# tinganchen/AlignQ

Hardware: AMD Instinct MI355X
Metric: images/sec (train step, CDF+ADMM) ResNet-20 8-bit (higher is better)
Workload: dtype f32; 1 GPU; resnet20 CIFAR-shape 3x32x32, 8W/8A CDF+ADMM full train step (cdf_alignment_admm/resnet-20-cifar-10), batch 128/GPU, HIP-graph replay, batch-norm folded into the site kernels, channels-last tensors, all Conv2d_Q convolutions on alignq_conv*_nhwc (exact-product bf16 MFMA); global_batch=128, parallelism=dp1

## Files before the change

alignq_amd/csrc/conv_kernels.hip:

```cpp
#include <hip/hip_runtime.h>
#include <stdint.h>
#include <stdlib.h>

#include "../../include/alignq.h"
#include "site_internal.h"
#include "store_forms.h"
#include "wgrad_reduce_body.h"

namespace {

using namespace alignq_wgr;

typedef __bf16 bf16x8 __attribute__((ext_vector_type(8)));
typedef __bf16 bf16x4 __attribute__((ext_vector_type(4)));
typedef float f32x4 __attribute__((ext_vector_type(4)));
typedef short s16x4 __attribute__((ext_vector_type(4)));

#ifdef ALIGNQ_STAMPS
__device__ unsigned long long g_conv_stamps[64];
__device__ unsigned long long g_conv_blk[2][4096];
#define STAMP(on, i)                                                          \
  do {                                                                        \
    if ((on) && threadIdx.x == 0) g_conv_stamps[i] = wall_clock64();          \
  } while (0)
#define BSTAMP(which)                                                                          \
  do {                                                                                         \
    if (threadIdx.x == 0 && blockIdx.x < 4096) g_conv_blk[which][blockIdx.x] = wall_clock64(); \
  } while (0)
#else
#define STAMP(on, i) do { } while (0)
#define BSTAMP(which) do { } while (0)
#endif

__device__ __forceinline__ s16x4 tr_read(const __bf16* p) {
  return __builtin_amdgcn_ds_read_tr16_b64_v4i16((__attribute__((address_space(3))) s16x4*)(p));
}
__device__ __forceinline__ bf16x8 join8(s16x4 a, s16x4 b) {
  typedef short s16x8 __attribute__((ext_vector_type(8)));
  s16x8 v = {a[0], a[1], a[2], a[3], b[0], b[1], b[2], b[3]};
  return __builtin_bit_cast(bf16x8, v);
}


template <int xb>
__device__ __forceinline__ f32x4 fetch_act4(const float* __restrict__ x, int64_t off) {
  if constexpr (xb == 0) return *reinterpret_cast<const f32x4*>(x + off);
  if constexpr (xb == 2) {
    const s16x4 b = *reinterpret_cast<const s16x4*>(reinterpret_cast<const short*>(x) + off);
    return (f32x4){(float)b[0], (float)b[1], (float)b[2], (float)b[3]};
  }
  const char4 b = *reinterpret_cast<const char4*>(reinterpret_cast<const signed char*>(x) + off);
  return (f32x4){(float)b.x, (float)b.y, (float)b.z, (float)b.w};
}

struct BnLazy {
  const float* z;
  const float* ab;
  const float* save;
  const float* ktot;
  const float* part = nullptr;
  int n_tiles = 0, tile_f = 0;
  double inv_n = 1.0;
  float* dgamma = nullptr;
  float* dbeta = nullptr;
};

template <int C>
__device__ __forceinline__ void bn_totals_lds(const BnLazy& t, float* __restrict__ kt, bool publish) {
  static_assert(256 % C == 0, "thread -> (channel, group)");
  __shared__ double red[256][2];
  constexpr int G = 256 / C;
  const int tid = threadIdx.x;
  const int cp = C < t.tile_f ? C : t.tile_f;
  const int cyc = C / cp, cnt = t.n_tiles / cyc;
  const int c = tid % C, grp = tid / C;
  const int e = c % cp, t_first = c / cp;
  double s0 = 0, s1 = 0;
  constexpr int U = 16;
  for (int i0 = grp; i0 < cnt; i0 += G * U) {
    float2 v[U];
#pragma unroll
    for (int u = 0; u < U; u++) {
      const int i = i0 + u * G;
      const int ic = i < cnt ? i : cnt - 1;
      v[u] = *reinterpret_cast<const float2*>(t.part + ((int64_t)(ic * cyc + t_first) * cp + e) * 2);
    }
#pragma unroll
    for (int u = 0; u < U; u++) {
      if (i0 + u * G < cnt) { s0 += v[u].x; s1 += v[u].y; }
    }
  }
  red[tid][0] = s0;
  red[tid][1] = s1;
  __syncthreads();
  if (tid < C) {
    double t0 = 0, t1 = 0;
#pragma unroll
    for (int g = 0; g < G; g++) { t0 += red[g * C + tid][0]; t1 += red[g * C + tid][1]; }
    kt[tid] = (float)(t0 * t.inv_n);
    kt[C + tid] = (float)(t1 * t.inv_n);
    if (publish) {
      if (t.dbeta) t.dbeta[tid] = (float)t0;
      if (t.dgamma) t.dgamma[tid] = (float)t1;
    }
  }
  __syncthreads();
}

__device__ __forceinline__ float4 bn_lazy4(const float4& g, const float4& z, const float4& a, const float4& m, const float4& is,
                                           const float4& k0, const float4& k1) {
  float4 o;
  o.x = a.x * (g.x - k0.x - (z.x - m.x) * is.x * k1.x);
  o.y = a.y * (g.y - k0.y - (z.y - m.y) * is.y * k1.y);
  o.z = a.z * (g.z - k0.z - (z.z - m.z) * is.z * k1.z);
  o.w = a.w * (g.w - k0.w - (z.w - m.w) * is.w * k1.w);
  return o;
}

template <int C> constexpr int conv_cp() { return C == 16 ? 16 : (C == 32 ? 48 : C + 8); }
template <int C, int WD, int PT>
struct ConvLds {
  static constexpr int kBf16 = 3 * ((PT / WD) + 2) * (WD + 2) * conv_cp<C>();
};

template <int C, int WD, int PT, bool DGRAD, int XB = 0, bool IMG = false>
__device__ __forceinline__ void conv3x3_body(const float* __restrict__ x, const float* __restrict__ w,
                                             float* __restrict__ y, int H, int total_rows, float nlev, __bf16* lds,
                                             int block, const float* __restrict__ add,
                                             float* __restrict__ bn_part = nullptr, int n_wg = 0,
                                             BnLazy lazy = BnLazy{nullptr, nullptr, nullptr, nullptr}, float xlev = 1.0f) {
  static_assert(XB == 0 || !DGRAD, "the data gradient reads fp32 dy");
  constexpr int xb = XB;
  constexpr int TR = PT / WD;
  constexpr int NS = (9 * C + 31) / 32;
  constexpr int NCG = C / 16;
  constexpr int NPP = 4 / NCG;
  constexpr int NG = PT / 16;
  constexpr int LW = WD + 2;
  constexpr int CP = conv_cp<C>();
  constexpr int LROWS = TR + 2;
  constexpr int ARR = LROWS * LW * CP;
  static_assert(3 * ARR == ConvLds<C, WD, PT>::kBf16, "LDS size");
  __bf16* Xhi = lds;
  __bf16* Xmi = lds + ARR;
  __bf16* Xlo = lds + 2 * ARR;

  const int tid = threadIdx.x, lane = tid & 63, wv = tid >> 6;
  const int row0 = block * TR;
  const int img_lo = (row0 / H) * H, img_hi = img_lo + H;
  [[maybe_unused]] constexpr int SB = DGRAD ? 8 : 0;
  STAMP(block == 0, SB + 0);
  const int cog = wv % NCG, pp = wv / NCG;
  const int m = lane & 15, q = lane >> 4;
  bf16x8 ab[NS];
  {
    constexpr int C4 = C / 4;
    constexpr int N4 = LROWS * LW * C4;
    constexpr int NIT = (N4 + 255) / 256;
    float4 v[NIT];
#pragma unroll
    for (int it = 0; it < NIT; it++) {
      const int i = tid + 256 * it;
      const int c4 = i % C4, col = (i / C4) % LW, lr = i / (C4 * LW);
      const int grow = row0 + lr - 1;
      const bool ok = i < N4 && col >= 1 && col <= WD && grow >= img_lo && grow < img_hi && grow < total_rows;
      const int64_t off = ok ? ((int64_t)grow * WD + (col - 1)) * C + 4 * c4 : 0;
      const f32x4 ld = fetch_act4<XB>(x, off);
      v[it] = ok ? make_float4(ld[0], ld[1], ld[2], ld[3]) : make_float4(0.f, 0.f, 0.f, 0.f);
    }
    STAMP(block == 0, SB + 1);
    if (DGRAD && lazy.z) {
      float4 zz[NIT];
#pragma unroll
      for (int it = 0; it < NIT; it++) {
        const int i = tid + 256 * it;
        const int c4 = i % C4, col = (i / C4) % LW, lr = i / (C4 * LW);
        const int grow = row0 + lr - 1;
        const bool ok = i < N4 && col >= 1 && col <= WD && grow >= img_lo && grow < img_hi && grow < total_rows;
        zz[it] = *reinterpret_cast<const float4*>(lazy.z + (ok ? ((int64_t)grow * WD + (col - 1)) * C + 4 * c4 : 0));
      }
      const int c4t = tid % C4;
      const float4 a4 = *reinterpret_cast<const float4*>(lazy.ab + 4 * c4t);
      const float4 m4 = *reinterpret_cast<const float4*>(lazy.save + 4 * c4t);
      const float4 i4 = *reinterpret_cast<const float4*>(lazy.save + C + 4 * c4t);
      float4 k0, k1;
      if (lazy.part) {
        __shared__ __attribute__((aligned(16))) float kt[2 * C];
        bn_totals_lds<C>(lazy, kt, block == 0);
        k0 = *reinterpret_cast<const float4*>(kt + 4 * c4t);
        k1 = *reinterpret_cast<const float4*>(kt + C + 4 * c4t);
      } else {
        k0 = *reinterpret_cast<const float4*>(lazy.ktot + 4 * c4t);
        k1 = *reinterpret_cast<const float4*>(lazy.ktot + C + 4 * c4t);
      }
#pragma unroll
      for (int it = 0; it < NIT; it++) {
        const int i = tid + 256 * it;
        const int col = (i / C4) % LW, lr = i / (C4 * LW);
        const int grow = row0 + lr - 1;
        const bool ok = i < N4 && col >= 1 && col <= WD && grow >= img_lo && grow < img_hi && grow < total_rows;
        if (ok) v[it] = bn_lazy4(v[it], zz[it], a4, m4, i4, k0, k1);
      }
    }
#pragma unroll
    for (int it = 0; it < NIT; it++) {
      const int i = tid + 256 * it;
      if (i < N4) {
        const int c4 = i % C4, col = (i / C4) % LW, lr = i / (C4 * LW);
        bf16x4 h4, m4, l4;
        const float vv[4] = {v[it].x, v[it].y, v[it].z, v[it].w};
#pragma unroll
        for (int e = 0; e < 4; e++) {
          const __bf16 hi = (__bf16)vv[e];
          const float r1 = vv[e] - (float)hi;
          const __bf16 mi = (__bf16)r1;
          const float r2 = r1 - (float)mi;
          h4[e] = hi; m4[e] = mi; l4[e] = (__bf16)r2;
        }
        const int o = (lr * LW + col) * CP + 4 * c4;
        *reinterpret_cast<bf16x4*>(Xhi + o) = h4;
        *reinterpret_cast<bf16x4*>(Xmi + o) = m4;
        *reinterpret_cast<bf16x4*>(Xlo + o) = l4;
      }
    }
    STAMP(block == 0, SB + 2);
    if constexpr (IMG) {
      const bf16x8* __restrict__ wi = reinterpret_cast<const bf16x8*>(w) + (cog * NS) * 64 + lane;
#pragma unroll
      for (int s = 0; s < NS; s++) ab[s] = wi[s * 64];
    } else {
#pragma unroll
      for (int s = 0; s < NS; s++) {
        const int k0 = 32 * s + 8 * q;
        const bool live = k0 / C < 9;
        const int tap = live ? k0 / C : 8, c0 = k0 % C;
        float wr[8];
        if (!DGRAD) {
          const float* p = w + ((int64_t)(cog * 16 + m) * 9 + tap) * C + c0;
          const float4 a4 = *reinterpret_cast<const float4*>(p), b4 = *reinterpret_cast<const float4*>(p + 4);
          wr[0] = a4.x; wr[1] = a4.y; wr[2] = a4.z; wr[3] = a4.w; wr[4] = b4.x; wr[5] = b4.y; wr[6] = b4.z; wr[7] = b4.w;
        } else {
#pragma unroll
          for (int j = 0; j < 8; j++) wr[j] = w[((int64_t)(c0 + j) * 9 + (8 - tap)) * C + cog * 16 + m];
        }
#pragma unroll
        for (int j = 0; j < 8; j++) ab[s][j] = (__bf16)rintf((live ? wr[j] : 0.f) * nlev);
      }
    }
    STAMP(block == 0, SB + 3);
  }
  __syncthreads();
  constexpr int GW = NG / NPP;
  static_assert(NG % NPP == 0, "every wave takes the same number of pixel groups");
  int bo[GW];
  f32x4 acc[GW];
#pragma unroll
  for (int gi = 0; gi < GW; gi++) {
    const int p = (pp + gi * NPP) * 16 + (lane & 15);
    bo[gi] = ((p / WD) * LW + (p % WD)) * CP;
    acc[gi] = (f32x4){0.f, 0.f, 0.f, 0.f};
  }
  constexpr int GB = (DGRAD && GW > 2) ? 2 : GW;
  static_assert(GW % GB == 0, "whole batches of groups");
#pragma unroll
  for (int g0 = 0; g0 < GW; g0 += GB) {
    bf16x8 bh[2][GB], bm[2][GB], bl[2][GB];
#pragma unroll
    for (int s = 0; s <= NS; s++) {
      if (s < NS) {
        const int k0 = 32 * s + 8 * q;
        const bool live = k0 / C < 9;
        const int tap = live ? k0 / C : 8, c0 = k0 % C;
        const int to = ((tap / 3) * LW + (tap % 3)) * CP + c0;
#pragma unroll
        for (int gi = 0; gi < GB; gi++) {
          const int o = bo[g0 + gi] + to;
          bh[s & 1][gi] = *reinterpret_cast<const bf16x8*>(Xhi + o);
          bm[s & 1][gi] = *reinterpret_cast<const bf16x8*>(Xmi + o);
          if (DGRAD || xb == 0) bl[s & 1][gi] = *reinterpret_cast<const bf16x8*>(Xlo + o);
          if ((9 * C) % 32 != 0 && !live) {
#pragma unroll
            for (int j = 0; j < 8; j++) { bh[s & 1][gi][j] = (__bf16)0.f; bm[s & 1][gi][j] = (__bf16)0.f; bl[s & 1][gi][j] = (__bf16)0.f; }
          }
        }
      }
      __builtin_amdgcn_sched_barrier(0);
      if (s > 0) {
        const int u = s - 1;
#pragma unroll
        for (int gi = 0; gi < GB; gi++) {
          f32x4 a = acc[g0 + gi];
          if (DGRAD || xb == 0) a = __builtin_amdgcn_mfma_f32_16x16x32_bf16(ab[u], bl[u & 1][gi], a, 0, 0, 0);
          a = __builtin_amdgcn_mfma_f32_16x16x32_bf16(ab[u], bm[u & 1][gi], a, 0, 0, 0);
          acc[g0 + gi] = __builtin_amdgcn_mfma_f32_16x16x32_bf16(ab[u], bh[u & 1][gi], a, 0, 0, 0);
        }
      }
    }
  }
  float bs[4] = {0.f, 0.f, 0.f, 0.f}, bq[4] = {0.f, 0.f, 0.f, 0.f};
#pragma unroll
  for (int gi = 0; gi < GW; gi++) {
    const int p = (pp + gi * NPP) * 16 + (lane & 15);
    const int r = p / WD, c = p % WD;
    const int grow = row0 + r;
    if (grow < total_rows) {
      const int64_t o = ((int64_t)grow * WD + c) * C + cog * 16 + 4 * q;
      const float den = (!DGRAD && xb != 0) ? nlev * xlev : nlev;
      float4 v = make_float4(acc[gi][0] / den, acc[gi][1] / den, acc[gi][2] / den, acc[gi][3] / den);
      if (add) {
        const float4 r = *reinterpret_cast<const float4*>(add + o);
        v.x += r.x; v.y += r.y; v.z += r.z; v.w += r.w;
      }
      alignq_store::st16<alignq_store::kConvOut>(y + o, v);
      bs[0] += v.x; bs[1] += v.y; bs[2] += v.z; bs[3] += v.w;
      bq[0] += v.x * v.x; bq[1] += v.y * v.y; bq[2] += v.z * v.z; bq[3] += v.w * v.w;
    }
  }
  STAMP(block == 0, SB + 4);
  if (!DGRAD && bn_part) {
    float* red = reinterpret_cast<float*>(lds);
#define ROW_SHR_ADD(V, CTRL) V += __builtin_bit_cast(float, __builtin_amdgcn_update_dpp(0, __builtin_bit_cast(int, V), CTRL, 0xf, 0xf, false))
#pragma unroll
    for (int e = 0; e < 4; e++) {
      ROW_SHR_ADD(bs[e], 0x111); ROW_SHR_ADD(bs[e], 0x112); ROW_SHR_ADD(bs[e], 0x114); ROW_SHR_ADD(bs[e], 0x118);
      ROW_SHR_ADD(bq[e], 0x111); ROW_SHR_ADD(bq[e], 0x112); ROW_SHR_ADD(bq[e], 0x114); ROW_SHR_ADD(bq[e], 0x118);
    }
#undef ROW_SHR_ADD
    __syncthreads();
    if ((lane & 15) == 15) {
#pragma unroll
      for (int e = 0; e < 4; e++) {
        red[(wv * 16 + 4 * q + e) * 2] = bs[e];
        red[(wv * 16 + 4 * q + e) * 2 + 1] = bq[e];
      }
    }
    __syncthreads();
    if (tid < C) {
      const int cg = tid / 16, cl = tid % 16;
      float s0 = 0.f, s1 = 0.f;
#pragma unroll
      for (int ppi = 0; ppi < NPP; ppi++) {
        const int w2 = ppi * NCG + cg;
        s0 += red[(w2 * 16 + cl) * 2];
        s1 += red[(w2 * 16 + cl) * 2 + 1];
      }
      bn_part[((int64_t)tid * n_wg + block) * 2] = s0;
      bn_part[((int64_t)tid * n_wg + block) * 2 + 1] = s1;
    }
  }
  STAMP(block == 0, SB + 5);
}

template <int C, int WD, int PT, bool DGRAD, int XB = 0, bool IMG = false>
__global__ __launch_bounds__(256) void conv3x3_nhwc_kernel(const float* __restrict__ x, const float* __restrict__ w,
                                                           float* __restrict__ y, int H, int total_rows, float nlev,
                                                           const float* __restrict__ add, float* __restrict__ bn_part,
                                                           float xlev) {
  __shared__ __attribute__((aligned(16))) __bf16 lds[ConvLds<C, WD, PT>::kBf16];
  conv3x3_body<C, WD, PT, DGRAD, XB, IMG>(x, w, y, H, total_rows, nlev, lds, blockIdx.x, add, bn_part, gridDim.x,
                                          BnLazy{nullptr, nullptr, nullptr, nullptr}, xlev);
}

template <int CIN, int COUT, int WDI, int KS, int S, int PT>
struct ConvGen {
  static constexpr int WDO = WDI / S, TR = PT / WDO;
  static constexpr int LROWS = KS == 3 ? TR * S + (S == 1 ? 2 : 1) : TR;
  static constexpr int LW = KS == 3 ? WDI + 2 : WDO;
  static constexpr int CP = CIN + 8;
  static constexpr int ARR = LROWS * LW * CP;
};

template <int CIN, int COUT, int WDI, int KS, int S, int PT, bool IMG = false>
__device__ __forceinline__ void convgen_fwd_body(const float* __restrict__ x, const float* __restrict__ w,
                                                 float* __restrict__ y, int H, int total_rows, float nlev,
                                                 float* __restrict__ bn_part, __bf16* lds, int block, int n_wg) {
  using G = ConvGen<CIN, COUT, WDI, KS, S, PT>;
  constexpr int WDO = G::WDO, TR = G::TR, LROWS = G::LROWS, LW = G::LW, CP = G::CP, ARR = G::ARR;
  constexpr int NS = (KS * KS * CIN + 31) / 32;
  constexpr int NCG = COUT / 16, NPP = 4 / NCG, NG = PT / 16;
  static_assert(NCG == 1 || NCG == 2 || NCG == 4, "output channels");
  __bf16* Xhi = lds;
  __bf16* Xmi = lds + ARR;
  __bf16* Xlo = lds + 2 * ARR;
  const int tid = threadIdx.x, lane = tid & 63, wv = tid >> 6;
  const int row0 = block * TR;
  const int Hin = H * S;
  const int img_lo = (row0 / H) * Hin, img_hi = img_lo + Hin;
  const int cog = wv % NCG, pp = wv / NCG;
  const int m = lane & 15, q = lane >> 4;
  bf16x8 ab[NS];
  {
    constexpr int C4 = CIN / 4;
    constexpr int N4 = LROWS * LW * C4;
    constexpr int NIT = (N4 + 255) / 256;
    float4 v[NIT];
#pragma unroll
    for (int it = 0; it < NIT; it++) {
      const int i = tid + 256 * it;
      const int c4 = i % C4, col = (i / C4) % LW, lr = i / (C4 * LW);
      int grow, gcol;
      if (KS == 3) { grow = row0 * S - 1 + lr; gcol = col - 1; }
      else { grow = (row0 + lr) * S; gcol = col * S; }
      const bool ok = i < N4 && gcol >= 0 && gcol < WDI && grow >= img_lo && grow < img_hi;
      v[it] = *reinterpret_cast<const float4*>(x + (ok ? ((int64_t)grow * WDI + gcol) * CIN + 4 * c4 : 0));
      if (!ok) v[it] = make_float4(0.f, 0.f, 0.f, 0.f);
    }
#pragma unroll
    for (int it = 0; it < NIT; it++) {
      const int i = tid + 256 * it;
      if (i < N4) {
        const int c4 = i % C4, col = (i / C4) % LW, lr = i / (C4 * LW);
        bf16x4 h4, m4, l4;
        const float vv[4] = {v[it].x, v[it].y, v[it].z, v[it].w};
#pragma unroll
        for (int e = 0; e < 4; e++) {
          const __bf16 hi = (__bf16)vv[e];
          const float r1 = vv[e] - (float)hi;
          const __bf16 mi = (__bf16)r1;
          h4[e] = hi; m4[e] = mi; l4[e] = (__bf16)(r1 - (float)mi);
        }
        const int o = (lr * LW + col) * CP + 4 * c4;
        *reinterpret_cast<bf16x4*>(Xhi + o) = h4;
        *reinterpret_cast<bf16x4*>(Xmi + o) = m4;
        *reinterpret_cast<bf16x4*>(Xlo + o) = l4;
      }
    }
    if constexpr (IMG) {
      const bf16x8* __restrict__ wi = reinterpret_cast<const bf16x8*>(w) + (cog * NS) * 64 + lane;
#pragma unroll
      for (int s = 0; s < NS; s++) ab[s] = wi[s * 64];
    } else {
#pragma unroll
      for (int s = 0; s < NS; s++) {
        const int k0 = 32 * s + 8 * q;
        const bool live = k0 / CIN < KS * KS;
        const int tap = live ? k0 / CIN : KS * KS - 1, c0 = k0 % CIN;
        const float* p = w + ((int64_t)(cog * 16 + m) * (KS * KS) + tap) * CIN + c0;
        const float4 a4 = *reinterpret_cast<const float4*>(p), b4 = *reinterpret_cast<const float4*>(p + 4);
        const float wr[8] = {a4.x, a4.y, a4.z, a4.w, b4.x, b4.y, b4.z, b4.w};
#pragma unroll
        for (int j = 0; j < 8; j++) ab[s][j] = (__bf16)rintf((live ? wr[j] : 0.f) * nlev);
      }
    }
  }
  __syncthreads();
  constexpr int GW = NG / NPP;
  static_assert(NG % NPP == 0, "every wave takes the same number of pixel groups");
  int bo[GW];
  f32x4 acc[GW];
#pragma unroll
  for (int gi = 0; gi < GW; gi++) {
    const int p = (pp + gi * NPP) * 16 + (lane & 15);
    const int r = p / WDO, c = p % WDO;
    bo[gi] = (KS == 3 ? (r * S * LW + c * S) : (r * LW + c)) * CP;
    acc[gi] = (f32x4){0.f, 0.f, 0.f, 0.f};
  }
  bf16x8 bh[2][GW], bm[2][GW], bl[2][GW];
#pragma unroll
  for (int s = 0; s <= NS; s++) {
    if (s < NS) {
      const int k0 = 32 * s + 8 * q;
      const bool live = k0 / CIN < KS * KS;
      const int tap = live ? k0 / CIN : KS * KS - 1, c0 = k0 % CIN;
      const int to = (KS == 3 ? ((tap / KS) * LW + (tap % KS)) * CP : 0) + c0;
#pragma unroll
      for (int gi = 0; gi < GW; gi++) {
        const int o = bo[gi] + to;
        bh[s & 1][gi] = *reinterpret_cast<const bf16x8*>(Xhi + o);
        bm[s & 1][gi] = *reinterpret_cast<const bf16x8*>(Xmi + o);
        bl[s & 1][gi] = *reinterpret_cast<const bf16x8*>(Xlo + o);
        if ((KS * KS * CIN) % 32 != 0 && !live) {
#pragma unroll
          for (int j = 0; j < 8; j++) { bh[s & 1][gi][j] = (__bf16)0.f; bm[s & 1][gi][j] = (__bf16)0.f; bl[s & 1][gi][j] = (__bf16)0.f; }
        }
      }
    }
    __builtin_amdgcn_sched_barrier(0);
    if (s > 0) {
      const int u = s - 1;
#pragma unroll
      for (int gi = 0; gi < GW; gi++) {
        f32x4 a = acc[gi];
        a = __builtin_amdgcn_mfma_f32_16x16x32_bf16(ab[u], bl[u & 1][gi], a, 0, 0, 0);
        a = __builtin_amdgcn_mfma_f32_16x16x32_bf16(ab[u], bm[u & 1][gi], a, 0, 0, 0);
        acc[gi] = __builtin_amdgcn_mfma_f32_16x16x32_bf16(ab[u], bh[u & 1][gi], a, 0, 0, 0);
      }
    }
  }
  float bs[4] = {0.f, 0.f, 0.f, 0.f}, bq[4] = {0.f, 0.f, 0.f, 0.f};
#pragma unroll
  for (int gi = 0; gi < GW; gi++) {
    const int p = (pp + gi * NPP) * 16 + (lane & 15);
    const int r = p / WDO, c = p % WDO;
    const int grow = row0 + r;
    if (grow < total_rows) {
      const float4 v = make_float4(acc[gi][0] / nlev, acc[gi][1] / nlev, acc[gi][2] / nlev, acc[gi][3] / nlev);
      alignq_store::st16<alignq_store::kConvOut>(y + ((int64_t)grow * WDO + c) * COUT + cog * 16 + 4 * q, v);
      bs[0] += v.x; bs[1] += v.y; bs[2] += v.z; bs[3] += v.w;
      bq[0] += v.x * v.x; bq[1] += v.y * v.y; bq[2] += v.z * v.z; bq[3] += v.w * v.w;
    }
  }
  if (bn_part) {
    float* red = reinterpret_cast<float*>(lds);
#define ROW_SHR_ADD(V, CTRL) V += __builtin_bit_cast(float, __builtin_amdgcn_update_dpp(0, __builtin_bit_cast(int, V), CTRL, 0xf, 0xf, false))
#pragma unroll
    for (int e = 0; e < 4; e++) {
      ROW_SHR_ADD(bs[e], 0x111); ROW_SHR_ADD(bs[e], 0x112); ROW_SHR_ADD(bs[e], 0x114); ROW_SHR_ADD(bs[e], 0x118);
      ROW_SHR_ADD(bq[e], 0x111); ROW_SHR_ADD(bq[e], 0x112); ROW_SHR_ADD(bq[e], 0x114); ROW_SHR_ADD(bq[e], 0x118);
    }
#undef ROW_SHR_ADD
    __syncthreads();
    if ((lane & 15) == 15) {
#pragma unroll
      for (int e = 0; e < 4; e++) {
        red[(wv * 16 + 4 * q + e) * 2] = bs[e];
        red[(wv * 16 + 4 * q + e) * 2 + 1] = bq[e];
      }
    }
    __syncthreads();
    if (tid < COUT) {
      const int cg = tid / 16, cl = tid % 16;
      float s0 = 0.f, s1 = 0.f;
#pragma unroll
      for (int ppi = 0; ppi < NPP; ppi++) {
        s0 += red[((ppi * NCG + cg) * 16 + cl) * 2];
        s1 += red[((ppi * NCG + cg) * 16 + cl) * 2 + 1];
      }
      bn_part[((int64_t)tid * n_wg + block) * 2] = s0;
      bn_part[((int64_t)tid * n_wg + block) * 2 + 1] = s1;
    }
  }
}

template <int CIN, int COUT, int WDI, int KS, int S, int PT, bool IMG = false>
__global__ __launch_bounds__(256) void convgen_fwd_kernel(const float* __restrict__ x, const float* __restrict__ w,
                                                          float* __restrict__ y, int H, int total_rows, float nlev,
                                                          float* __restrict__ bn_part) {
  __shared__ __attribute__((aligned(16))) __bf16 lds[3 * ConvGen<CIN, COUT, WDI, KS, S, PT>::ARR];
  convgen_fwd_body<CIN, COUT, WDI, KS, S, PT, IMG>(x, w, y, H, total_rows, nlev, bn_part, lds, blockIdx.x, gridDim.x);
}

template <int CIN, int COUT, int WDI, int PT3, int PT1, bool IMG = false>
__global__ __launch_bounds__(256) void transition_fwd_kernel(const float* __restrict__ x, const float* __restrict__ w3,
                                                             const float* __restrict__ w1, float* __restrict__ y3,
                                                             float* __restrict__ y1, int H, int total_rows, float nlev,
                                                             float* __restrict__ part3, float* __restrict__ part1, int n3) {
  constexpr int A3 = ConvGen<CIN, COUT, WDI, 3, 2, PT3>::ARR, A1 = ConvGen<CIN, COUT, WDI, 1, 2, PT1>::ARR;
  __shared__ __attribute__((aligned(16))) __bf16 lds[3 * (A3 > A1 ? A3 : A1)];
  if ((int)blockIdx.x < n3)
    convgen_fwd_body<CIN, COUT, WDI, 3, 2, PT3, IMG>(x, w3, y3, H, total_rows, nlev, part3, lds, blockIdx.x, n3);
  else
    convgen_fwd_body<CIN, COUT, WDI, 1, 2, PT1, IMG>(x, w1, y1, H, total_rows, nlev, part1, lds, blockIdx.x - n3,
                                                     (int)gridDim.x - n3);
}

template <int CIN, int COUT, int WDI, int KS, int PT, bool WITH1, bool IMG = false>
__device__ __forceinline__ void dgrad_s2_body(const float* __restrict__ dy, const float* __restrict__ w,
                                              float* __restrict__ dx, int H, int total_rows, float nlev,
                                              const float* __restrict__ add, BnLazy lazy, __bf16* lds, int block,
                                              const float* __restrict__ dy1 = nullptr, const float* __restrict__ w1 = nullptr,
                                              BnLazy lazy1 = BnLazy{nullptr, nullptr, nullptr, nullptr}) {
  static_assert(!WITH1 || KS == 3, "the second source is the 1x1 shortcut of a 3x3 transition");
  constexpr int P = KS == 3 ? 1 : 0;
  constexpr int WDO = WDI / 2, TR = PT / WDI;
  constexpr int DROWS = TR / 2 + P, DCOLS = WDO + P;
  constexpr int CP = COUT + 8;
  constexpr int NPIX3 = DROWS * DCOLS + 1;
  constexpr int NPIX1 = WITH1 ? (TR / 2) * WDO : 0;
  constexpr int NPIX = NPIX3 + NPIX1;
  constexpr int ARR = NPIX * CP;
  constexpr int NT = KS * KS + (WITH1 ? 1 : 0);
  constexpr int NS = (NT * COUT + 31) / 32;
  constexpr int NCG = CIN / 16, NPP = 4 / NCG, NG = PT / 16;
  __bf16* Xhi = lds;
  __bf16* Xmi = lds + ARR;
  __bf16* Xlo = lds + 2 * ARR;
  const int tid = threadIdx.x, lane = tid & 63, wv = tid >> 6;
  const int row0 = block * TR;
  const int Ho = H / 2;
  const int orow0 = (row0 / H) * Ho + (row0 % H) / 2;
  const int oimg_hi = (row0 / H + 1) * Ho;
  {
    constexpr int C4 = COUT / 4;
    constexpr int N4 = NPIX3 * C4;
    constexpr int NIT = (N4 + 255) / 256;
    constexpr int M4 = NPIX1 * C4;
    constexpr int NI1 = WITH1 ? (M4 + 255) / 256 : 1;
    float4 v[NIT], zz[NIT], v1[NI1], z1[NI1];
#pragma unroll
    for (int it = 0; it < NIT; it++) {
      const int i = tid + 256 * it;
      const int c4 = i % C4, pix = i / C4;
      const int lr = pix / DCOLS, col = pix % DCOLS;
      const int grow = orow0 + lr;
      const bool ok = i < N4 && pix < DROWS * DCOLS && col < WDO && grow < oimg_hi;
      const int64_t off = ok ? ((int64_t)grow * WDO + col) * COUT + 4 * c4 : 0;
      v[it] = *reinterpret_cast<const float4*>(dy + off);
      if (lazy.z) zz[it] = *reinterpret_cast<const float4*>(lazy.z + off);
      if (!ok) v[it] = make_float4(0.f, 0.f, 0.f, 0.f);
    }
    if constexpr (WITH1) {
#pragma unroll
      for (int it = 0; it < NI1; it++) {
        const int i = tid + 256 * it;
        const int64_t off = i < M4 ? ((int64_t)orow0 * WDO) * COUT + 4 * (int64_t)i : 0;
        v1[it] = *reinterpret_cast<const float4*>(dy1 + off);
        if (lazy1.z) z1[it] = *reinterpret_cast<const float4*>(lazy1.z + off);
      }
    }
    const int c4t = tid % C4;
    if (lazy.z) {
      const float4 a4 = *reinterpret_cast<const float4*>(lazy.ab + 4 * c4t);
      const float4 m4 = *reinterpret_cast<const float4*>(lazy.save + 4 * c4t);
      const float4 i4 = *reinterpret_cast<const float4*>(lazy.save + COUT + 4 * c4t);
      float4 k0, k1;
      if (lazy.part) {
        __shared__ __attribute__((aligned(16))) float kt[2 * COUT];
        bn_totals_lds<COUT>(lazy, kt, block == 0);
        k0 = *reinterpret_cast<const float4*>(kt + 4 * c4t);
        k1 = *reinterpret_cast<const float4*>(kt + COUT + 4 * c4t);
      } else {
        k0 = *reinterpret_cast<const float4*>(lazy.ktot + 4 * c4t);
        k1 = *reinterpret_cast<const float4*>(lazy.ktot + COUT + 4 * c4t);
      }
#pragma unroll
      for (int it = 0; it < NIT; it++) {
        const int i = tid + 256 * it;
        const int pix = i / C4;
        const int lr = pix / DCOLS, col = pix % DCOLS;
        const bool ok = i < N4 && pix < DROWS * DCOLS && col < WDO && orow0 + lr < oimg_hi;
        if (ok) v[it] = bn_lazy4(v[it], zz[it], a4, m4, i4, k0, k1);
      }
    }
    if constexpr (WITH1) {
      if (lazy1.z) {
        const float4 a4 = *reinterpret_cast<const float4*>(lazy1.ab + 4 * c4t);
        const float4 m4 = *reinterpret_cast<const float4*>(lazy1.save + 4 * c4t);
        const float4 i4 = *reinterpret_cast<const float4*>(lazy1.save + COUT + 4 * c4t);
        float4 k0, k1;
        if (lazy1.part) {
          __shared__ __attribute__((aligned(16))) float kt1[2 * COUT];
          bn_totals_lds<COUT>(lazy1, kt1, block == 0);
          k0 = *reinterpret_cast<const float4*>(kt1 + 4 * c4t);
          k1 = *reinterpret_cast<const float4*>(kt1 + COUT + 4 * c4t);
        } else {
          k0 = *reinterpret_cast<const float4*>(lazy1.ktot + 4 * c4t);
          k1 = *reinterpret_cast<const float4*>(lazy1.ktot + COUT + 4 * c4t);
        }
#pragma unroll
        for (int it = 0; it < NI1; it++) {
          if (tid + 256 * it < M4) v1[it] = bn_lazy4(v1[it], z1[it], a4, m4, i4, k0, k1);
        }
      }
    }
#pragma unroll
    for (int it = 0; it < NIT + (WITH1 ? NI1 : 0); it++) {
      const bool second = it >= NIT;
      const int i = tid + 256 * (second ? it - NIT : it);
      if (i < (second ? M4 : N4)) {
        const int c4 = i % C4, pix = (second ? NPIX3 : 0) + i / C4;
        bf16x4 h4, m4, l4;
        const float4 src = second ? v1[second ? it - NIT : 0] : v[second ? 0 : it];
        const float vv[4] = {src.x, src.y, src.z, src.w};
#pragma unroll
        for (int e = 0; e < 4; e++) {
          const __bf16 hi = (__bf16)vv[e];
          const float r1 = vv[e] - (float)hi;
          const __bf16 mi = (__bf16)r1;
          h4[e] = hi; m4[e] = mi; l4[e] = (__bf16)(r1 - (float)mi);
        }
        const int o = pix * CP + 4 * c4;
        *reinterpret_cast<bf16x4*>(Xhi + o) = h4;
        *reinterpret_cast<bf16x4*>(Xmi + o) = m4;
        *reinterpret_cast<bf16x4*>(Xlo + o) = l4;
      }
    }
  }
  const int cig = wv % NCG, pp = wv / NCG;
  const int m = lane & 15, q = lane >> 4;
  bf16x8 ab[NS];
  if constexpr (IMG) {
    static_assert((KS * KS * COUT) % 32 == 0 && COUT % 32 == 0, "whole k steps per filter");
    constexpr int NS3 = KS * KS * COUT / 32;
    const bf16x8* __restrict__ wi = reinterpret_cast<const bf16x8*>(w) + (cig * NS3) * 64 + lane;
#pragma unroll
    for (int s = 0; s < NS3; s++) ab[s] = wi[s * 64];
    if constexpr (WITH1) {
      const bf16x8* __restrict__ wj = reinterpret_cast<const bf16x8*>(w1) + (cig * (NS - NS3)) * 64 + lane;
#pragma unroll
      for (int s = NS3; s < NS; s++) ab[s] = wj[(s - NS3) * 64];
    }
  } else {
#pragma unroll
    for (int s = 0; s < NS; s++) {
      const int k0 = 32 * s + 8 * q;
      const int tap = k0 / COUT, c0 = k0 % COUT;
#pragma unroll
      for (int j = 0; j < 8; j++) {
        float v = 0.f;
        if (tap < KS * KS) v = w[((int64_t)(c0 + j) * (KS * KS) + tap) * CIN + cig * 16 + m];
        else if (WITH1 && tap == KS * KS) v = w1[(int64_t)(c0 + j) * CIN + cig * 16 + m];
        ab[s][j] = (__bf16)rintf(v * nlev);
      }
    }
  }
  __syncthreads();
  for (int g = pp; g < NG; g += NPP) {
    const int p = g * 16 + (lane & 15);
    const int r = p / WDI, c = p % WDI;
    f32x4 acc = {0.f, 0.f, 0.f, 0.f};
#pragma unroll
    for (int s = 0; s < NS; s++) {
      const int k0 = 32 * s + 8 * q;
      const int tap = k0 / COUT, c0 = k0 % COUT;
      int pix = DROWS * DCOLS;
      if (tap < KS * KS) {
        const int ky = tap / KS, kx = tap % KS;
        const int a = r + P - ky, b = c + P - kx;
        if (a >= 0 && b >= 0 && !(a & 1) && !(b & 1)) pix = (a >> 1) * DCOLS + (b >> 1);
      } else if (WITH1 && tap == KS * KS) {
        if (!(r & 1) && !(c & 1)) pix = NPIX3 + (r >> 1) * WDO + (c >> 1);
      }
      const int o = pix * CP + c0;
      const bf16x8 bh = *reinterpret_cast<const bf16x8*>(Xhi + o);
      const bf16x8 bm = *reinterpret_cast<const bf16x8*>(Xmi + o);
      const bf16x8 bl = *reinterpret_cast<const bf16x8*>(Xlo + o);
      acc = __builtin_amdgcn_mfma_f32_16x16x32_bf16(ab[s], bl, acc, 0, 0, 0);
      acc = __builtin_amdgcn_mfma_f32_16x16x32_bf16(ab[s], bm, acc, 0, 0, 0);
      acc = __builtin_amdgcn_mfma_f32_16x16x32_bf16(ab[s], bh, acc, 0, 0, 0);
    }
    const int grow = row0 + r;
    if (grow < total_rows) {
      const int64_t o = ((int64_t)grow * WDI + c) * CIN + cig * 16 + 4 * q;
      float4 out = make_float4(acc[0] / nlev, acc[1] / nlev, acc[2] / nlev, acc[3] / nlev);
      if (add) {
        const float4 a4 = *reinterpret_cast<const float4*>(add + o);
        out.x += a4.x; out.y += a4.y; out.z += a4.z; out.w += a4.w;
      }
      alignq_store::st16<alignq_store::kConvOut>(dx + o, out);
    }
  }
}

template <int CIN, int COUT, int WDI, int KS, int PT, bool WITH1>
struct DgradS2Lds {
  static constexpr int P = KS == 3 ? 1 : 0, TR = PT / WDI;
  static constexpr int kBf16 = 3 * (((TR / 2 + P) * (WDI / 2 + P) + 1) + (WITH1 ? (TR / 2) * (WDI / 2) : 0)) * (COUT + 8);
};

template <int CIN, int COUT, int WDI, int KS, int PT, bool IMG = false>
__global__ __launch_bounds__(256) void dgrad_s2_kernel(const float* __restrict__ dy, const float* __restrict__ w,
                                                       float* __restrict__ dx, int H, int total_rows, float nlev,
                                                       const float* __restrict__ add, BnLazy lazy) {
  __shared__ __attribute__((aligned(16))) __bf16 lds[DgradS2Lds<CIN, COUT, WDI, KS, PT, false>::kBf16];
  dgrad_s2_body<CIN, COUT, WDI, KS, PT, false, IMG>(dy, w, dx, H, total_rows, nlev, add, lazy, lds, blockIdx.x);
}

template <int CIN, int COUT, int WDI, int KS, int PT>
int launch_dgrad_s2(const float* dy, const float* w, float* dx, int B, int H, float nlev, const float* add, BnLazy lazy,
                    hipStream_t st, bool img = false) {
  constexpr int TR = PT / WDI;
  static_assert(TR % 2 == 0, "even number of input rows per tile");
  if (H % TR) return ALIGNQ_EUNSUPPORTED;
  const int total_rows = B * H;
  if (img)
    hipLaunchKernelGGL((dgrad_s2_kernel<CIN, COUT, WDI, KS, PT, true>), total_rows / TR, 256, 0, st, dy, w, dx, H, total_rows, nlev,
                       add, lazy);
  else
    hipLaunchKernelGGL((dgrad_s2_kernel<CIN, COUT, WDI, KS, PT>), total_rows / TR, 256, 0, st, dy, w, dx, H, total_rows, nlev,
                       add, lazy);
  hipError_t e = hipGetLastError();
  return e == hipSuccess ? 0 : (int)e;
}

constexpr int kStemPT = 128;
__device__ __forceinline__ void stem_stage(const float* __restrict__ x, int H, int row0, __bf16* Chi, __bf16* Cmi, __bf16* Clo) {
  const int tid = threadIdx.x;
  const int pix = tid >> 1, half = tid & 1;
  const int r = pix / 32, c = pix % 32;
  const int grow = row0 + r;
  const int ih = grow % H;
  float v[16];
#pragma unroll
  for (int j = 0; j < 16; j++) {
    const int k = 16 * half + j;
    const int tap = k / 3, ci = k % 3;
    const int ky = tap / 3, kx = tap % 3;
    const int yy = ih + ky - 1, xx = c + kx - 1;
    const bool ok = k < 27 && yy >= 0 && yy < H && xx >= 0 && xx < 32;
    v[j] = x[ok ? ((int64_t)(grow + ky - 1) * 32 + xx) * 3 + ci : 0];
    if (!ok) v[j] = 0.f;
  }
  bf16x8 h[2], m[2], l[2];
#pragma unroll
  for (int j = 0; j < 16; j++) {
    const __bf16 hi = (__bf16)v[j];
    const float r1 = v[j] - (float)hi;
    const __bf16 mi = (__bf16)r1;
    h[j >> 3][j & 7] = hi; m[j >> 3][j & 7] = mi; l[j >> 3][j & 7] = (__bf16)(r1 - (float)mi);
  }
  const int o = pix * 32 + 16 * half;
  *reinterpret_cast<bf16x8*>(Chi + o) = h[0]; *reinterpret_cast<bf16x8*>(Chi + o + 8) = h[1];
  *reinterpret_cast<bf16x8*>(Cmi + o) = m[0]; *reinterpret_cast<bf16x8*>(Cmi + o + 8) = m[1];
  *reinterpret_cast<bf16x8*>(Clo + o) = l[0]; *reinterpret_cast<bf16x8*>(Clo + o + 8) = l[1];
}

__global__ __launch_bounds__(256) void stem_fwd_kernel(const float* __restrict__ x, const float* __restrict__ w,
                                                       float* __restrict__ y, int H, int total_rows, float nlev,
                                                       float* __restrict__ bn_part) {
  __shared__ __attribute__((aligned(16))) __bf16 lds[3 * kStemPT * 32];
  __bf16* Chi = lds;
  __bf16* Cmi = lds + kStemPT * 32;
  __bf16* Clo = lds + 2 * kStemPT * 32;
  const int tid = threadIdx.x, lane = tid & 63, wv = tid >> 6;
  const int row0 = blockIdx.x * 4;
  stem_stage(x, H, row0, Chi, Cmi, Clo);
  const int m = lane & 15, q = lane >> 4;
  bf16x8 ab;
#pragma unroll
  for (int j = 0; j < 8; j++) {
    const int k = 8 * q + j;
    ab[j] = (__bf16)rintf((k < 27 ? w[m * 27 + k] : 0.f) * nlev);
  }
  __syncthreads();
  float bs[4] = {0.f, 0.f, 0.f, 0.f}, bq[4] = {0.f, 0.f, 0.f, 0.f};
  for (int g = wv; g < kStemPT / 16; g += 4) {
    const int p = g * 16 + (lane & 15);
    const int o = p * 32 + 8 * q;
    f32x4 acc = {0.f, 0.f, 0.f, 0.f};
    acc = __builtin_amdgcn_mfma_f32_16x16x32_bf16(ab, *reinterpret_cast<const bf16x8*>(Clo + o), acc, 0, 0, 0);
    acc = __builtin_amdgcn_mfma_f32_16x16x32_bf16(ab, *reinterpret_cast<const bf16x8*>(Cmi + o), acc, 0, 0, 0);
    acc = __builtin_amdgcn_mfma_f32_16x16x32_bf16(ab, *reinterpret_cast<const bf16x8*>(Chi + o), acc, 0, 0, 0);
    const int grow = row0 + p / 32;
    if (grow < total_rows) {
      const float4 v = make_float4(acc[0] / nlev, acc[1] / nlev, acc[2] / nlev, acc[3] / nlev);
      alignq_store::st16<alignq_store::kConvOut>(y + ((int64_t)grow * 32 + p % 32) * 16 + 4 * q, v);
      bs[0] += v.x; bs[1] += v.y; bs[2] += v.z; bs[3] += v.w;
      bq[0] += v.x * v.x; bq[1] += v.y * v.y; bq[2] += v.z * v.z; bq[3] += v.w * v.w;
    }
  }
  if (bn_part) {
    float* red = reinterpret_cast<float*>(lds);
#define ROW_SHR_ADD(V, CTRL) V += __builtin_bit_cast(float, __builtin_amdgcn_update_dpp(0, __builtin_bit_cast(int, V), CTRL, 0xf, 0xf, false))
#pragma unroll
    for (int e = 0; e < 4; e++) {
      ROW_SHR_ADD(bs[e], 0x111); ROW_SHR_ADD(bs[e], 0x112); ROW_SHR_ADD(bs[e], 0x114); ROW_SHR_ADD(bs[e], 0x118);
      ROW_SHR_ADD(bq[e], 0x111); ROW_SHR_ADD(bq[e], 0x112); ROW_SHR_ADD(bq[e], 0x114); ROW_SHR_ADD(bq[e], 0x118);
    }
#undef ROW_SHR_ADD
    __syncthreads();
    if ((lane & 15) == 15) {
#pragma unroll
      for (int e = 0; e < 4; e++) {
        red[(wv * 16 + 4 * q + e) * 2] = bs[e];
        red[(wv * 16 + 4 * q + e) * 2 + 1] = bq[e];
      }
    }
    __syncthreads();
    if (tid < 16) {
      float s0 = 0.f, s1 = 0.f;
#pragma unroll
      for (int w2 = 0; w2 < 4; w2++) { s0 += red[(w2 * 16 + tid) * 2]; s1 += red[(w2 * 16 + tid) * 2 + 1]; }
      bn_part[((int64_t)tid * gridDim.x + blockIdx.x) * 2] = s0;
      bn_part[((int64_t)tid * gridDim.x + blockIdx.x) * 2 + 1] = s1;
    }
  }
}

__global__ __launch_bounds__(256) void stem_wgrad_kernel(const float* __restrict__ x, const float* __restrict__ dy,
                                                         float* __restrict__ slabs, int H, int n_tiles, BnLazy lazy) {
  __shared__ __attribute__((aligned(16))) __bf16 lds[3 * kStemPT * 32 + 3 * kStemPT * 16];
  __bf16* Ci[3] = {lds, lds + kStemPT * 32, lds + 2 * kStemPT * 32};
  __bf16* Di[3] = {lds + 3 * kStemPT * 32, lds + 3 * kStemPT * 32 + kStemPT * 16, lds + 3 * kStemPT * 32 + 2 * kStemPT * 16};
  const int tid = threadIdx.x, lane = tid & 63, wv = tid >> 6;
  const int g = lane >> 4, q = (lane & 15) >> 2, pcol = 4 * (lane & 3);
  f32x4 acc[2] = {{0.f, 0.f, 0.f, 0.f}, {0.f, 0.f, 0.f, 0.f}};
  __shared__ __attribute__((aligned(16))) float kt[32];
  if (lazy.z && lazy.part) bn_totals_lds<16>(lazy, kt, blockIdx.x == 0);
  for (int tile = blockIdx.x; tile < n_tiles; tile += gridDim.x) {
    const int row0 = tile * 4;
    f32x4 dvr[2], zvr[2];
#pragma unroll
    for (int it = 0; it < 2; it++) {
      const int i = tid + 256 * it;
      const int64_t off = ((int64_t)row0 * 32 + i / 4) * 16 + 4 * (tid % 4);
      dvr[it] = *reinterpret_cast<const f32x4*>(dy + off);
      zvr[it] = lazy.z ? *reinterpret_cast<const f32x4*>(lazy.z + off) : (f32x4){0.f, 0.f, 0.f, 0.f};
    }
    __syncthreads();
    stem_stage(x, H, row0, Ci[0], Ci[1], Ci[2]);
    {
      const int c4 = tid % 4;
      f32x4 la = {0, 0, 0, 0}, lm = la, li = la, lk0 = la, lk1 = la;
      if (lazy.z) {
        la = *reinterpret_cast<const f32x4*>(lazy.ab + 4 * c4);
        lm = *reinterpret_cast<const f32x4*>(lazy.save + 4 * c4);
        li = *reinterpret_cast<const f32x4*>(lazy.save + 16 + 4 * c4);
        const float* kp = lazy.part ? kt : lazy.ktot;
        lk0 = *reinterpret_cast<const f32x4*>(kp + 4 * c4);
        lk1 = *reinterpret_cast<const f32x4*>(kp + 16 + 4 * c4);
      }
#pragma unroll
      for (int it = 0; it < 2; it++) {
        const int i = tid + 256 * it;
        f32x4 dv = dvr[it];
        if (lazy.z) dv = la * (dv - lk0 - (zvr[it] - lm) * li * lk1);
        bf16x4 h4, m4, l4;
#pragma unroll
        for (int e = 0; e < 4; e++) {
          const __bf16 hi = (__bf16)dv[e];
          const float r1 = dv[e] - (float)hi;
          const __bf16 mi = (__bf16)r1;
          h4[e] = hi; m4[e] = mi; l4[e] = (__bf16)(r1 - (float)mi);
        }
        const int o = (i / 4) * 16 + 4 * c4;
        *reinterpret_cast<bf16x4*>(Di[0] + o) = h4;
        *reinterpret_cast<bf16x4*>(Di[1] + o) = m4;
        *reinterpret_cast<bf16x4*>(Di[2] + o) = l4;
      }
    }
    __syncthreads();
    {
      const int p0 = 32 * wv + 8 * g;
      bf16x8 a[3];
#pragma unroll
      for (int t = 0; t < 3; t++) {
        const __bf16* pa = Di[t] + (p0 + q) * 16 + pcol;
        a[t] = join8(tr_read(pa), tr_read(pa + 4 * 16));
      }
#pragma unroll
      for (int blk = 0; blk < 2; blk++) {
        bf16x8 b[3];
#pragma unroll
        for (int t = 0; t < 3; t++) {
          const __bf16* pb = Ci[t] + (p0 + q) * 32 + 16 * blk + pcol;
          b[t] = join8(tr_read(pb), tr_read(pb + 4 * 32));
        }
        f32x4 v = acc[blk];
        v = __builtin_amdgcn_mfma_f32_16x16x32_bf16(a[1], b[1], v, 0, 0, 0);
        v = __builtin_amdgcn_mfma_f32_16x16x32_bf16(a[0], b[2], v, 0, 0, 0);
        v = __builtin_amdgcn_mfma_f32_16x16x32_bf16(a[2], b[0], v, 0, 0, 0);
        v = __builtin_amdgcn_mfma_f32_16x16x32_bf16(a[0], b[1], v, 0, 0, 0);
        v = __builtin_amdgcn_mfma_f32_16x16x32_bf16(a[1], b[0], v, 0, 0, 0);
        v = __builtin_amdgcn_mfma_f32_16x16x32_bf16(a[0], b[0], v, 0, 0, 0);
        acc[blk] = v;
      }
    }
  }
  float* red = reinterpret_cast<float*>(lds);
  __syncthreads();
  if (wv > 0) {
#pragma unroll
    for (int blk = 0; blk < 2; blk++)
#pragma unroll
      for (int e = 0; e < 4; e++) red[(((wv - 1) * 2 + blk) * 4 + e) * 64 + lane] = acc[blk][e];
  }
  __syncthreads();
  if (wv == 0) {
    float* slab = slabs + (int64_t)blockIdx.x * (16 * 27);
#pragma unroll
    for (int blk = 0; blk < 2; blk++) {
#pragma unroll
      for (int e = 0; e < 4; e++) {
        float v = acc[blk][e];
#pragma unroll
        for (int w2 = 0; w2 < 3; w2++) v += red[((w2 * 2 + blk) * 4 + e) * 64 + lane];
        const int k = 16 * blk + (lane & 15), co = 4 * (lane >> 4) + e;
        if (k < 27) slab[co * 27 + k] = v;
      }
    }
  }
}

template <int CIN, int COUT, int WDI, int KS, int S, int PT>
int launch_gen(const float* x, const float* w, float* y, int B, int H, float nlev, float* bn_part, hipStream_t st,
               bool img = false) {
  constexpr int TR = ConvGen<CIN, COUT, WDI, KS, S, PT>::TR;
  if (H % TR) return ALIGNQ_EUNSUPPORTED;
  const int total_rows = B * H;
  if (img)
    hipLaunchKernelGGL((convgen_fwd_kernel<CIN, COUT, WDI, KS, S, PT, true>), total_rows / TR, 256, 0, st, x, w, y, H, total_rows,
                       nlev, bn_part);
  else
    hipLaunchKernelGGL((convgen_fwd_kernel<CIN, COUT, WDI, KS, S, PT>), total_rows / TR, 256, 0, st, x, w, y, H, total_rows,
                       nlev, bn_part);
  hipError_t e = hipGetLastError();
  return e == hipSuccess ? 0 : (int)e;
}

template <int C, int WD, int PT>
int launch(const float* x, const float* w, float* y, int B, int H, int dgrad, float nlev, const float* add, float* bn_part,
           hipStream_t st, int xb = 0, float xlev = 1.0f, bool img = false) {
  constexpr int TR = PT / WD;
  const int total_rows = B * H;
  if (H % TR) return ALIGNQ_EUNSUPPORTED;
  const int grid = total_rows / TR;
  if (img) {
    if (dgrad) hipLaunchKernelGGL((conv3x3_nhwc_kernel<C, WD, PT, true, 0, true>), grid, 256, 0, st, x, w, y, H, total_rows, nlev, add, nullptr, 1.0f);
    else if (xb == 2) hipLaunchKernelGGL((conv3x3_nhwc_kernel<C, WD, PT, false, 2, true>), grid, 256, 0, st, x, w, y, H, total_rows, nlev, add, bn_part, xlev);
    else if (xb == 1) hipLaunchKernelGGL((conv3x3_nhwc_kernel<C, WD, PT, false, 1, true>), grid, 256, 0, st, x, w, y, H, total_rows, nlev, add, bn_part, xlev);
    else hipLaunchKernelGGL((conv3x3_nhwc_kernel<C, WD, PT, false, 0, true>), grid, 256, 0, st, x, w, y, H, total_rows, nlev, add, bn_part, xlev);
  } else if (dgrad) hipLaunchKernelGGL((conv3x3_nhwc_kernel<C, WD, PT, true, 0>), grid, 256, 0, st, x, w, y, H, total_rows, nlev, add, nullptr, 1.0f);
  else if (xb == 2) hipLaunchKernelGGL((conv3x3_nhwc_kernel<C, WD, PT, false, 2>), grid, 256, 0, st, x, w, y, H, total_rows, nlev, add, bn_part, xlev);
  else if (xb == 1) hipLaunchKernelGGL((conv3x3_nhwc_kernel<C, WD, PT, false, 1>), grid, 256, 0, st, x, w, y, H, total_rows, nlev, add, bn_part, xlev);
  else hipLaunchKernelGGL((conv3x3_nhwc_kernel<C, WD, PT, false, 0>), grid, 256, 0, st, x, w, y, H, total_rows, nlev, add, bn_part, xlev);
  hipError_t e = hipGetLastError();
  return e == hipSuccess ? 0 : (int)e;
}

typedef float f32x16 __attribute__((ext_vector_type(16)));

template <int CIN, int COUT, int WDI, int KS, int S, int PT>
struct WgradGeo {
  static constexpr int WDO = WDI / S, TR = PT / WDO, NT = KS * KS;
  static constexpr int CB = (CIN < COUT ? CIN : COUT) >= 32 ? 32 : 16;
  static constexpr int XROWS = KS == 3 ? TR * S + (S == 1 ? 2 : 1) : TR;
  static constexpr int LW = KS == 3 ? WDI + 2 : WDO;
  static constexpr int XA = XROWS * LW * CB;
  static constexpr int DA = PT * CB;
  static constexpr int kRed = 3 * NT * 4 * 64 * 4;
  static constexpr int kBytes = (3 * (XA + DA) * 2) > kRed ? (3 * (XA + DA) * 2) : kRed;
  static constexpr int kFloats = kBytes / 4;
};
template <int C, int WD, int PT>
struct WgradLds : WgradGeo<C, C, WD, 3, 1, PT> {};

template <int CIN, int COUT, int WDI, int KS, int S, int PT, int XB = 0>
__device__ __forceinline__ void wgrad_body(const float* __restrict__ x, const float* __restrict__ dy,
                                           float* __restrict__ slabs, int H, int n_tiles, float* lds_f, int bx, int gx,
                                           int by, BnLazy lazy = BnLazy{nullptr, nullptr, nullptr, nullptr}, float xlev = 1.0f) {
  constexpr int xb = XB;
  using G = WgradGeo<CIN, COUT, WDI, KS, S, PT>;
  constexpr int WDO = G::WDO, TR = G::TR, NT = G::NT, CB = G::CB, LW = G::LW, XA = G::XA, DA = G::DA, XROWS = G::XROWS;
  constexpr int NBLK = CIN / CB;
  constexpr int NSTEP = PT / 32;
  static_assert(WDO % 8 == 0 && PT % 32 == 0, "a lane group's 8 pixels lie in one output row");
  __bf16* lds = reinterpret_cast<__bf16*>(lds_f);
  __bf16* Xi[3] = {lds, lds + XA, lds + 2 * XA};
  __bf16* Di[3] = {lds + 3 * XA, lds + 3 * XA + DA, lds + 3 * XA + 2 * DA};
  const int tid = threadIdx.x, lane = tid & 63, wv = tid >> 6;
  const int bi = by / NBLK, bj = by % NBLK;
  const int cob = CB == 32 ? (wv >> 1) : 0, cib = CB == 32 ? (wv & 1) : 0;
  const int g = lane >> 4, q = (lane & 15) >> 2, pcol = 4 * (lane & 3);

// ... 841 lines not shown
```

Measured before the change: 141,300 images/sec.

## Split stride-2 dgrad into parity classes to skip zero-tap MFMAs

The stride-2 transposed-conv gradient loop now handles output pixels in four compile-time parity classes. Each class statically drops the kernel taps that hit no input for that parity, instead of issuing MFMAs against a zero pixel. This removes roughly three quarters of the wasted MFMA and LDS reads for 3x3 taps, at the cost of four specialised loop bodies and more code size. A separate change unrolls the first pass of the C=32 BN-totals reduction twice as deep, and debug stamps (compiled out by default) are added.

```diff
diff --git a/alignq_amd/csrc/conv_kernels.hip b/alignq_amd/csrc/conv_kernels.hip
--- a/alignq_amd/csrc/conv_kernels.hip
+++ b/alignq_amd/csrc/conv_kernels.hip
@@ -1,6 +1,8 @@
 #include <hip/hip_runtime.h>
 #include <stdint.h>
 #include <stdlib.h>
+
+#include <type_traits>
 
 #include "../../include/alignq.h"
 #include "site_internal.h"
@@ -77,7 +79,25 @@
   const int e = c % cp, t_first = c / cp;
   double s0 = 0, s1 = 0;
   constexpr int U = 16;
-  for (int i0 = grp; i0 < cnt; i0 += G * U) {
+  int i_next = grp;
+  if constexpr (C == 32) {
+    if (cnt > G * U) {
+      constexpr int U2 = 2 * U;
+      float2 v[U2];
+#pragma unroll
+      for (int u = 0; u < U2; u++) {
+        const int i = grp + u * G;
+        const int ic = i < cnt ? i : cnt - 1;
+        v[u] = *reinterpret_cast<const float2*>(t.part + ((int64_t)(ic * cyc + t_first) * cp + e) * 2);
+      }
+#pragma unroll
+      for (int u = 0; u < U2; u++) {
+        if (grp + u * G < cnt) { s0 += v[u].x; s1 += v[u].y; }
+      }
+      i_next = grp + G * U2;
+    }
+  }
+  for (int i0 = i_next; i0 < cnt; i0 += G * U) {
     float2 v[U];
 #pragma unroll
     for (int u = 0; u < U; u++) {
@@ -571,7 +591,8 @@
   constexpr int ARR = NPIX * CP;
   constexpr int NT = KS * KS + (WITH1 ? 1 : 0);
   constexpr int NS = (NT * COUT + 31) / 32;
-  constexpr int NCG = CIN / 16, NPP = 4 / NCG, NG = PT / 16;
+  constexpr int NCG = CIN / 16, NPP = 4 / NCG;
+  static_assert((NPP & (NPP - 1)) == 0, "wave -> unit round-robin");
   __bf16* Xhi = lds;
   __bf16* Xmi = lds + ARR;
   __bf16* Xlo = lds + 2 * ARR;
@@ -580,6 +601,7 @@
   const int Ho = H / 2;
   const int orow0 = (row0 / H) * Ho + (row0 % H) / 2;
   const int oimg_hi = (row0 / H + 1) * Ho;
+  STAMP(block == 0, 56);
   {
     constexpr int C4 = COUT / 4;
     constexpr int N4 = NPIX3 * C4;
@@ -608,6 +630,7 @@
         if (lazy1.z) z1[it] = *reinterpret_cast<const float4*>(lazy1.z + off);
       }
     }
+    STAMP(block == 0, 57);
     const int c4t = tid % C4;
     if (lazy.z) {
       const float4 a4 = *reinterpret_cast<const float4*>(lazy.ab + 4 * c4t);
@@ -705,41 +728,55 @@
     }
   }
   __syncthreads();
-  for (int g = pp; g < NG; g += NPP) {
-    const int p = g * 16 + (lane & 15);
-    const int r = p / WDI, c = p % WDI;
-    f32x4 acc = {0.f, 0.f, 0.f, 0.f};
-#pragma unroll
-    for (int s = 0; s < NS; s++) {
-      const int k0 = 32 * s + 8 * q;
-      const int tap = k0 / COUT, c0 = k0 % COUT;
-      int pix = DROWS * DCOLS;
-      if (tap < KS * KS) {
-        const int ky = tap / KS, kx = tap % KS;
-        const int a = r + P - ky, b = c + P - kx;
-        if (a >= 0 && b >= 0 && !(a & 1) && !(b & 1)) pix = (a >> 1) * DCOLS + (b >> 1);
-      } else if (WITH1 && tap == KS * KS) {
-        if (!(r & 1) && !(c & 1)) pix = NPIX3 + (r >> 1) * WDO + (c >> 1);
-      }
-      const int o = pix * CP + c0;
-      const bf16x8 bh = *reinterpret_cast<const bf16x8*>(Xhi + o);
-      const bf16x8 bm = *reinterpret_cast<const bf16x8*>(Xmi + o);
-      const bf16x8 bl = *reinterpret_cast<const bf16x8*>(Xlo + o);
-      acc = __builtin_amdgcn_mfma_f32_16x16x32_bf16(ab[s], bl, acc, 0, 0, 0);
-      acc = __builtin_amdgcn_mfma_f32_16x16x32_bf16(ab[s], bm, acc, 0, 0, 0);
-      acc = __builtin_amdgcn_mfma_f32_16x16x32_bf16(ab[s], bh, acc, 0, 0, 0);
-    }
-    const int grow = row0 + r;
-    if (grow < total_rows) {
-      const int64_t o = ((int64_t)grow * WDI + c) * CIN + cig * 16 + 4 * q;
-      float4 out = make_float4(acc[0] / nlev, acc[1] / nlev, acc[2] / nlev, acc[3] / nlev);
-      if (add) {
-        const float4 a4 = *reinterpret_cast<const float4*>(add + o);
-        out.x += a4.x; out.y += a4.y; out.z += a4.z; out.w += a4.w;
-      }
-      alignq_store::st16<alignq_store::kConvOut>(dx + o, out);
-    }
-  }
+  STAMP(block == 0, 58);
+  constexpr int HW = WDI / 2;
+  constexpr int NGC = PT / 64;
+  static_assert(PT % 64 == 0 && (HW & (HW - 1)) == 0 && COUT % 32 == 0, "whole groups per class, whole k steps per tap");
+  auto run_class = [&](auto cls_c) {
+    constexpr int CLS = decltype(cls_c)::value;
+    constexpr int RP = CLS >> 1, CQ = CLS & 1;
+    for (int gc = (pp - CLS * NGC) & (NPP - 1); gc < NGC; gc += NPP) {
+      const int idx = gc * 16 + (lane & 15);
+      const int rr = idx / HW, cc = idx % HW;
+      const int r = 2 * rr + RP, c = 2 * cc + CQ;
+      const int o3 = (rr * DCOLS + cc) * CP + 8 * q;
+      [[maybe_unused]] const int o1 = (NPIX3 + rr * WDO + cc) * CP + 8 * q;
+      f32x4 acc = {0.f, 0.f, 0.f, 0.f};
+#pragma unroll
+      for (int s = 0; s < NS; s++) {
+        const int tap = 32 * s / COUT, c0 = 32 * s % COUT;
+        int o = -1;
+        if (tap < KS * KS) {
+          const int da = RP + P - tap / KS, db = CQ + P - tap % KS;
+          if (!(da & 1) && !(db & 1)) o = o3 + ((da / 2) * DCOLS + db / 2) * CP + c0;
+        } else if (WITH1 && tap == KS * KS) {
+          if (RP == 0 && CQ == 0) o = o1 + c0;
+        }
+        if (o < 0) continue;
+        const bf16x8 bh = *reinterpret_cast<const bf16x8*>(Xhi + o);
+        const bf16x8 bm = *reinterpret_cast<const bf16x8*>(Xmi + o);
+        const bf16x8 bl = *reinterpret_cast<const bf16x8*>(Xlo + o);
+        acc = __builtin_amdgcn_mfma_f32_16x16x32_bf16(ab[s], bl, acc, 0, 0, 0);
+        acc = __builtin_amdgcn_mfma_f32_16x16x32_bf16(ab[s], bm, acc, 0, 0, 0);
+        acc = __builtin_amdgcn_mfma_f32_16x16x32_bf16(ab[s], bh, acc, 0, 0, 0);
+      }
+      const int grow = row0 + r;
+      if (grow < total_rows) {
+        const int64_t o = ((int64_t)grow * WDI + c) * CIN + cig * 16 + 4 * q;
+        float4 out = make_float4(acc[0] / nlev, acc[1] / nlev, acc[2] / nlev, acc[3] / nlev);
+        if (add) {
+          const float4 a4 = *reinterpret_cast<const float4*>(add + o);
+          out.x += a4.x; out.y += a4.y; out.z += a4.z; out.w += a4.w;
+        }
+        alignq_store::st16<alignq_store::kConvOut>(dx + o, out);
+      }
+    }
+  };
+  run_class(std::integral_constant<int, 0>{});
+  run_class(std::integral_constant<int, 1>{});
+  run_class(std::integral_constant<int, 2>{});
+  run_class(std::integral_constant<int, 3>{});
+  STAMP(block == 0, 59);
 }
 
 template <int CIN, int COUT, int WDI, int KS, int PT, bool WITH1>
```

After: 142,000 images/sec, median of 4. Within noise of the previous version (+0.6%).
